# LauraFJulia/TFT_vs_Fund

Measured on NVIDIA B200. Metric: 3-view linear TFT pose solves/sec (LinearTFTPoseEstimation + ReprError, n=20), higher is better.
Workload: dtype f64

## Files before the change

### tft_vs_fund_b200/csrc/tvf_math.cuh

```cuda
#pragma once
#include <math.h>

#if defined(__CUDACC__)
#define TVF_HD __host__ __device__ __forceinline__
#else
#define TVF_HD inline
#endif

namespace tvf {

#ifndef TVF_FAST_RSQRT
#define TVF_FAST_RSQRT 1
#endif
#ifndef TVF_DLT_PREDICT
#define TVF_DLT_PREDICT 1
#endif

TVF_HD double rsqrt_(double x) {
#if defined(__CUDA_ARCH__)
#if TVF_FAST_RSQRT
    double y;
    asm("rsqrt.approx.ftz.f64 %0, %1;" : "=d"(y) : "d"(x));
    const double h = 0.5 * x;
    double e = fma(-h * y, y, 0.5);
// ... 183 lines not shown
    const double tiny = 1e-300 + 1e-18 * rmax;
    double d[3];
#pragma unroll
    for (int k = 0; k < 3; ++k) {
        const double p = (fabs(rr[k][k]) < tiny) ? copysign(tiny, rr[k][k]) : rr[k][k];
        d[k] = rcp_(p);
    }
    double x2 = d[2];
    double x1 = -(rr[1][2] * x2) * d[1];
    double x0 = -(rr[0][1] * x1 + rr[0][2] * x2) * d[0];
    double inv = rsqrt_(x0 * x0 + x1 * x1 + x2 * x2);
    x0 *= inv; x1 *= inv; x2 *= inv;
    double dprev = 0.0;
    bool ok = false;
    for (int it = 0; it < NULL3_MAX_IT; ++it) {
        const double y0 = x0 * d[0];
        const double y1 = (x1 - rr[0][1] * y0) * d[1];
        const double y2 = (x2 - rr[0][2] * y0 - rr[1][2] * y1) * d[2];
        double z2 = y2 * d[2];
        double z1 = (y1 - rr[1][2] * z2) * d[1];
        double z0 = (y0 - rr[0][1] * z1 - rr[0][2] * z2) * d[0];
        inv = rsqrt_(z0 * z0 + z1 * z1 + z2 * z2);
        z0 *= inv; z1 *= inv; z2 *= inv;
        const double e0 = z0 - x0, e1 = z1 - x1, e2 = z2 - x2;
        const double d2 = e0 * e0 + e1 * e1 + e2 * e2;
        x0 = z0; x1 = z1; x2 = z2;
        if (!(d2 > 1e-26) || !(d2 * d2 > 1e-28 * dprev)) { ok = (d2 == d2); break; }
        dprev = d2;
    }
    v[0] = x0; v[1] = x1; v[2] = x2;
    return ok;
}

TVF_HD void null3(const double* M, double* v) {
#if TVF_NULL3_QR
    if (null3_qr(M, false, v)) return;
#endif
    double A[9], V[9], s[3];
#pragma unroll
    for (int i = 0; i < 9; ++i) A[i] = M[i];
    jacobi_svd3(A, V, s);
    v[0] = V[6]; v[1] = V[7]; v[2] = V[8];
}
TVF_HD void null3_t(const double* M, double* v) {
#if TVF_NULL3_QR
    if (null3_qr(M, true, v)) return;
#endif
    double A[9], V[9], s[3];
#pragma unroll
    for (int c = 0; c < 3; ++c)
#pragma unroll
        for (int r = 0; r < 3; ++r) A[r + 3 * c] = M[c + 3 * r];
    jacobi_svd3(A, V, s);
    v[0] = V[6]; v[1] = V[7]; v[2] = V[8];
}

TVF_HD void svd3_full(const double* M, double* U, double* s, double* V) {
    double A[9];
#pragma unroll
    for (int i = 0; i < 9; ++i) A[i] = M[i];
    jacobi_svd3(A, V, s);
    const double i0 = rcp_(s[0]), i1 = rcp_(s[1]);
#pragma unroll
    for (int i = 0; i < 3; ++i) { U[i] = A[i] * i0; U[3 + i] = A[3 + i] * i1; }
    cross3(U, U + 3, U + 6);
}

TVF_HD void epipole_from_nulls(const double* v0, const double* v1, const double* v2, double* e) {
    double M[9];
#pragma unroll
    for (int c = 0; c < 3; ++c) { M[0 + 3 * c] = v0[c]; M[1 + 3 * c] = v1[c]; M[2 + 3 * c] = v2[c]; }
    null3(M, e);
}

TVF_HD void tft_epipoles(const double* T, double* e21, double* e31) {
    double v[9];
    null3(T, v); null3(T + 9, v + 3); null3(T + 18, v + 6);
    epipole_from_nulls(v, v + 3, v + 6, e31);
    null3_t(T, v); null3_t(T + 9, v + 3); null3_t(T + 18, v + 6);
    epipole_from_nulls(v, v + 3, v + 6, e21);
}

TVF_HD void onb3(const double* e, double* u1, double* u2) {
    const double sg = copysign(1.0, e[2]);
    const double a = -rcp_(sg + e[2]);
    const double b = e[0] * e[1] * a;
    u1[0] = 1.0 + sg * e[0] * e[0] * a; u1[1] = sg * b; u1[2] = -sg * e[0];
    u2[0] = b; u2[1] = sg + e[1] * e[1] * a; u2[2] = -e[1];
}

TVF_HD void transform_tft(const double* T, const double* M1, const double* M2, const double* M3,
                          int inverse, double* Tn) {
    double A1[9], A2[9], A3[9];
    if (inverse) {
#pragma unroll
        for (int i = 0; i < 9; ++i) A1[i] = M1[i];
        inv3(M2, A2); inv3(M3, A3);
    } else {
        inv3(M1, A1);
#pragma unroll
        for (int i = 0; i < 9; ++i) { A2[i] = M2[i]; A3[i] = M3[i]; }
    }
    double nrm = 0.0;
#pragma unroll
    for (int i = 0; i < 3; ++i) {
        double S[9], L[9];
#pragma unroll
        for (int e = 0; e < 9; ++e)
            S[e] = A1[0 + 3 * i] * T[e] + A1[1 + 3 * i] * T[9 + e] + A1[2 + 3 * i] * T[18 + e];
        mat3_mul(A2, S, L);
        mat3_mul_nt(L, A3, Tn + 9 * i);
#pragma unroll
        for (int e = 0; e < 9; ++e) nrm += Tn[9 * i + e] * Tn[9 * i + e];
    }
    const double inv = 1.0 / sqrt(nrm);
#pragma unroll
    for (int e = 0; e < 27; ++e) Tn[e] *= inv;
}

TVF_HD double det4_rows(const double* a, const double* b, const double* c, const double* d) {
    const double s0 = a[0] * b[1] - a[1] * b[0], s1 = a[0] * b[2] - a[2] * b[0];
    const double s2 = a[0] * b[3] - a[3] * b[0], s3 = a[1] * b[2] - a[2] * b[1];
    const double s4 = a[1] * b[3] - a[3] * b[1], s5 = a[2] * b[3] - a[3] * b[2];
    const double c5 = c[2] * d[3] - c[3] * d[2], c4 = c[1] * d[3] - c[3] * d[1];
    const double c3 = c[1] * d[2] - c[2] * d[1], c2 = c[0] * d[3] - c[3] * d[0];
    const double c1 = c[0] * d[2] - c[2] * d[0], c0 = c[0] * d[1] - c[1] * d[0];
    return s0 * c5 - s1 * c4 + s2 * c3 + s3 * c2 - s4 * c1 + s5 * c0;
}

TVF_HD void tft_from_p(const double* P1, const double* P2, const double* P3, double* T) {
    double r1[3][4], r2[3][4], r3[3][4];
#pragma unroll
    for (int r = 0; r < 3; ++r)
#pragma unroll
        for (int c = 0; c < 4; ++c) { r1[r][c] = P1[r + 3 * c]; r2[r][c] = P2[r + 3 * c]; r3[r][c] = P3[r + 3 * c]; }
    double nrm = 0.0;
#pragma unroll
    for (int i = 0; i < 3; ++i) {
        const int ra = (i == 0) ? 1 : 0, rb = (i == 2) ? 1 : 2;
        const double sg = (i == 1) ? -1.0 : 1.0;
#pragma unroll
        for (int j = 0; j < 3; ++j)
#pragma unroll
            for (int k = 0; k < 3; ++k) {
                const double d = sg * det4_rows(r1[ra], r1[rb], r2[j], r3[k]);
                T[j + 3 * k + 9 * i] = d; nrm += d * d;
            }
    }
    const double inv = 1.0 / sqrt(nrm);
#pragma unroll
    for (int e = 0; e < 27; ++e) T[e] *= inv;
}

template <int M>
TVF_HD void dlt_null(double (&a)[M][4], double* x, int* iters = nullptr) {
    double r[4][4];
#pragma unroll
    for (int k = 0; k < 4; ++k) {
        if (M == 4 && k == 3) {
            r[3][3] = -a[3][3];
            break;
        }
        double sig = 0.0;
#pragma unroll
        for (int i = k; i < M; ++i) sig += a[i][k] * a[i][k];
        const double nrm = sqrt_(sig);
        const double x1 = a[k][k];
        const double alpha = -copysign(nrm, x1);
        const double den = sig - alpha * x1;
        const double f = (den > 0.0) ? rcp_(den) : 0.0;
        const double vk = x1 - alpha;
#pragma unroll
        for (int c = k + 1; c < 4; ++c) {
            double sdot = vk * a[k][c];
#pragma unroll
            for (int i = k + 1; i < M; ++i) sdot += a[i][k] * a[i][c];
            sdot *= f;
            a[k][c] -= sdot * vk;
#pragma unroll
            for (int i = k + 1; i < M; ++i) a[i][c] -= sdot * a[i][k];
        }
        r[k][k] = alpha;
#pragma unroll
        for (int c = k + 1; c < 4; ++c) r[k][c] = a[k][c];
    }
    const double rmax = fmax(fmax(fabs(r[0][0]), fabs(r[1][1])), fmax(fabs(r[2][2]), fabs(r[3][3])));
    const double tiny = 1e-300 + 1e-18 * rmax;
    double d[4];
#pragma unroll
    for (int k = 0; k < 4; ++k) {
        const double p = (fabs(r[k][k]) < tiny) ? copysign(tiny, r[k][k]) : r[k][k];
        d[k] = rcp_(p);
    }
    double x0, x1, x2, x3;
    x3 = d[3];
    x2 = -(r[2][3] * x3) * d[2];
    x1 = -(r[1][2] * x2 + r[1][3] * x3) * d[1];
    x0 = -(r[0][1] * x1 + r[0][2] * x2 + r[0][3] * x3) * d[0];
    double inv = rsqrt_(x0 * x0 + x1 * x1 + x2 * x2 + x3 * x3);
    x0 *= inv; x1 *= inv; x2 *= inv; x3 *= inv;
    int it = 0;
#if TVF_DLT_PREDICT
    double dprev = 0.0;
#endif
    for (; it < 40; ++it) {
        const double y0 = x0 * d[0];
        const double y1 = (x1 - r[0][1] * y0) * d[1];
        const double y2 = (x2 - r[0][2] * y0 - r[1][2] * y1) * d[2];
        const double y3 = (x3 - r[0][3] * y0 - r[1][3] * y1 - r[2][3] * y2) * d[3];
        double z3 = y3 * d[3];
        double z2 = (y2 - r[2][3] * z3) * d[2];
        double z1 = (y1 - r[1][2] * z2 - r[1][3] * z3) * d[1];
        double z0 = (y0 - r[0][1] * z1 - r[0][2] * z2 - r[0][3] * z3) * d[0];
        inv = rsqrt_(z0 * z0 + z1 * z1 + z2 * z2 + z3 * z3);
        z0 *= inv; z1 *= inv; z2 *= inv; z3 *= inv;
#if TVF_DLT_PREDICT
        const double e0 = z0 - x0, e1 = z1 - x1, e2 = z2 - x2, e3 = z3 - x3;
        const double d2 = e0 * e0 + e1 * e1 + e2 * e2 + e3 * e3;
        x0 = z0; x1 = z1; x2 = z2; x3 = z3;
        if (!(d2 > 1e-26) || !(d2 * d2 > 1e-28 * dprev)) { ++it; break; }
        dprev = d2;
#else
        const double diff = fmax(fmax(fabs(z0 - x0), fabs(z1 - x1)), fmax(fabs(z2 - x2), fabs(z3 - x3)));
        x0 = z0; x1 = z1; x2 = z2; x3 = z3;
        if (!(diff > 1e-13)) { ++it; break; }
#endif
    }
    x[0] = x0; x[1] = x1; x[2] = x2; x[3] = x3;
    if (iters) *iters = it;
}

TVF_HD bool dlt4_depth_signs(const double (&a)[4][4], const double* r3, double tz, int* s_x, int* s_z) {
    double g[4][4];
#pragma unroll
    for (int i = 0; i < 4; ++i)
#pragma unroll
        for (int j = 0; j <= i; ++j) g[i][j] = a[0][i] * a[0][j] + a[1][i] * a[1][j] + a[2][i] * a[2][j] + a[3][i] * a[3][j];
    const double gmax = fmax(fmax(g[0][0], g[1][1]), fmax(g[2][2], g[3][3]));
    const double pmin = 1.0e-3 * gmax;
    if (!(g[0][0] >= pmin)) return false;
    const double i0 = rsqrt_(g[0][0]);
    const double l10 = g[1][0] * i0, l20 = g[2][0] * i0, l30 = g[3][0] * i0;
    const double p1 = g[1][1] - l10 * l10;
    if (!(p1 >= pmin)) return false;
    const double i1 = rsqrt_(p1);
    const double l21 = (g[2][1] - l20 * l10) * i1, l31 = (g[3][1] - l30 * l10) * i1;
    const double p2 = g[2][2] - l20 * l20 - l21 * l21;
    if (!(p2 >= pmin)) return false;
    const double i2 = rsqrt_(p2);
    const double l32 = (g[3][2] - l30 * l20 - l31 * l21) * i2;
    double p3 = g[3][3] - l30 * l30 - l31 * l31 - l32 * l32;
    p3 = (p3 >= 1.0e-14 * gmax) ? p3 : 1.0e-14 * gmax;
    const double i3 = rsqrt_(p3);
    double x3 = i3;
    double x2 = -(l32 * x3) * i2;
    double x1 = -(l21 * x2 + l31 * x3) * i1;
    double x0 = -(l10 * x1 + l20 * x2 + l30 * x3) * i0;
    double inv = rsqrt_(x0 * x0 + x1 * x1 + x2 * x2 + x3 * x3);
    x0 *= inv; x1 *= inv; x2 *= inv; x3 *= inv;
    double d2 = 1.0;
#pragma unroll
    for (int it = 0; it < 2; ++it) {
        const double y0 = x0 * i0;
        const double y1 = (x1 - l10 * y0) * i1;
        const double y2 = (x2 - l20 * y0 - l21 * y1) * i2;
        const double y3 = (x3 - l30 * y0 - l31 * y1 - l32 * y2) * i3;
        double z3 = y3 * i3;
        double z2 = (y2 - l32 * z3) * i2;
        double z1 = (y1 - l21 * z2 - l31 * z3) * i1;
        double z0 = (y0 - l10 * z1 - l20 * z2 - l30 * z3) * i0;
        inv = rsqrt_(z0 * z0 + z1 * z1 + z2 * z2 + z3 * z3);
        z0 *= inv; z1 *= inv; z2 *= inv; z3 *= inv;
        const double e0 = z0 - x0, e1 = z1 - x1, e2 = z2 - x2, e3 = z3 - x3;
        d2 = e0 * e0 + e1 * e1 + e2 * e2 + e3 * e3;
        x0 = z0; x1 = z1; x2 = z2; x3 = z3;
        if (d2 <= 1.0e-10) break;
    }
    if (!(d2 <= 1.0e-10)) return false;
    const double q1 = x2 * x3;
    const double zc = r3[0] * x0 + r3[1] * x1 + r3[2] * x2 + tz * x3;
    const double q2 = zc * x3;
    if (!(fabs(q1) >= 1.0e-3) || !(fabs(q2) >= 1.0e-3)) return false;
    *s_x = (q1 > 0.0) ? 1 : -1;
    *s_z = (q2 > 0.0) ? 1 : -1;
    return true;
}

template <bool AFF = false>
TVF_HD void dlt_row_minors(const double* ra, const double* rb, double* m7) {
    m7[0] = ra[0] * rb[1] - ra[1] * rb[0]; m7[1] = ra[0] * rb[2] - ra[2] * rb[0];
    m7[3] = ra[1] * rb[2] - ra[2] * rb[1];
    if (AFF) {
        m7[2] = 0.0; m7[4] = 0.0; m7[5] = 0.0;
        m7[6] = (ra[0] * ra[0] + ra[1] * ra[1] + ra[2] * ra[2]) + (rb[0] * rb[0] + rb[1] * rb[1] + rb[2] * rb[2]);
    } else {
        m7[2] = ra[0] * rb[3] - ra[3] * rb[0]; m7[4] = ra[1] * rb[3] - ra[3] * rb[1]; m7[5] = ra[2] * rb[3] - ra[3] * rb[2];
        m7[6] = (ra[0] * ra[0] + ra[1] * ra[1] + ra[2] * ra[2] + ra[3] * ra[3]) + (rb[0] * rb[0] + rb[1] * rb[1] + rb[2] * rb[2] + rb[3] * rb[3]);
    }
}
template <bool AFF = false>
TVF_HD bool dlt4_depth_signs_ray(const double* m7, const double* rc, const double* rd, const double* r3, double tz,
                                 int* s_x, int* s_z) {
    const double M01 = m7[0], M02 = m7[1], M03 = m7[2], M12 = m7[3], M13 = m7[4], M23 = m7[5];
    const double X0 = AFF ? rc[3] * M12 : rc[1] * M23 - rc[2] * M13 + rc[3] * M12;
    const double X1 = AFF ? -(rc[3] * M02) : -(rc[0] * M23 - rc[2] * M03 + rc[3] * M02);
    const double X2 = AFF ? rc[3] * M01 : rc[0] * M13 - rc[1] * M03 + rc[3] * M01;
    const double X3 = -(rc[0] * M12 - rc[1] * M02 + rc[2] * M01);
    const double xx = X0 * X0 + X1 * X1 + X2 * X2 + X3 * X3;
    const double b2 = m7[6] + (rc[0] * rc[0] + rc[1] * rc[1] + rc[2] * rc[2] + rc[3] * rc[3]);
    const double rho = rd[0] * X0 + rd[1] * X1 + rd[2] * X2 + rd[3] * X3;
    const double rb2 = fabs(rho) * b2;
    if (!(rb2 < 0.4 * xx)) return false;
    if (!(xx >= 1.0e-12 * (b2 * b2 * b2))) return false;
    const double q1 = X2 * X3;
    const double zc = r3[0] * X0 + r3[1] * X1 + r3[2] * X2 + tz * X3;
    const double q2 = zc * X3;
    const double floor_ = 1.0e-6 * xx;
    if (!(fabs(q1) >= 1.0605 * rb2 + floor_)) return false;
    if (!(fabs(q2) >= 1.616 * rb2 + floor_)) return false;
    *s_x = (q1 > 0.0) ? 1 : -1;
    *s_z = (q2 > 0.0) ? 1 : -1;
    return true;
}

TVF_HD void dlt_rows(const double* P, double x, double y, double* row_a, double* row_b) {
#pragma unroll
    for (int c = 0; c < 4; ++c) {
        row_a[c] = y * P[2 + 3 * c] - P[1 + 3 * c];
        row_b[c] = P[0 + 3 * c] - x * P[2 + 3 * c];
    }
}

TVF_HD void cam_apply(const double* P, const double* X, double* out) {
#pragma unroll
    for (int r = 0; r < 3; ++r)
        out[r] = P[r] * X[0] + P[r + 3] * X[1] + P[r + 6] * X[2] + P[r + 9] * X[3];
}

TVF_HD void decompose_essential(const double* E, double* R, double* Rp, double* t) {
    double U[9], s[3], V[9];
    svd3_full(E, U, s, V);
    double UW[9], UWt[9];
#pragma unroll
    for (int i = 0; i < 3; ++i) {
        UW[i] = U[3 + i]; UW[3 + i] = -U[i]; UW[6 + i] = U[6 + i];
        UWt[i] = -U[3 + i]; UWt[3 + i] = U[i]; UWt[6 + i] = U[6 + i];
    }
    mat3_mul_nt(UW, V, R);
    mat3_mul_nt(UWt, V, Rp);
    const double sr = sign_(det3(R)), sp = sign_(det3(Rp));
#pragma unroll
    for (int i = 0; i < 9; ++i) { R[i] *= sr; Rp[i] *= sp; }
    t[0] = U[6]; t[1] = U[7]; t[2] = U[8];
}

TVF_HD double matlab_abs_acos(double x) {
    if (x > 1.0) return log(x + sqrt(x * x - 1.0));
    if (x < -1.0) {
        const double a = log(-x + sqrt(x * x - 1.0));
        return sqrt(3.14159265358979323846 * 3.14159265358979323846 + a * a);
    }
    return acos(x);
}

TVF_HD void ang_error(const double* Rt_true, const double* Rt_est, double* rot_err, double* t_err) {
    double tr = 0.0;
#pragma unroll
    for (int i = 0; i < 9; ++i) tr += Rt_true[i] * Rt_est[i];
    const double k = 180.0 / 3.14159265358979323846;
    *rot_err = fabs(k * matlab_abs_acos((tr - 1.0) / 2.0));
    const double* a = Rt_est + 9; const double* b = Rt_true + 9;
    const double na = sqrt(a[0] * a[0] + a[1] * a[1] + a[2] * a[2]);
    const double nb = sqrt(b[0] * b[0] + b[1] * b[1] + b[2] * b[2]);
    const double d = (a[0] / na) * (b[0] / nb) + (a[1] / na) * (b[1] / nb) + (a[2] / na) * (b[2] / nb);
    *t_err = fabs(k * matlab_abs_acos(d));
}

}
```

### tft_vs_fund_b200/csrc/tvf_pose.cuh

```cuda
#pragma once
#include "tvf_math.cuh"

#ifndef TVF_CHEIR_UNROLL
#define TVF_CHEIR_UNROLL 1
#endif
#ifndef TVF_VOTE_FAST_SIGNS
#define TVF_VOTE_FAST_SIGNS 1
#endif
#ifndef TVF_VOTE_GRAM_SIGNS
#define TVF_VOTE_GRAM_SIGNS 0
#endif
#ifndef TVF_VOTE_RAY_SIGNS
#define TVF_VOTE_RAY_SIGNS 1
#endif
#ifndef TVF_CHEIR_NOINLINE
#define TVF_CHEIR_NOINLINE 0
#endif

namespace tvf {

constexpr int CAND_PAIR = 42;
constexpr int CAND_SIZE = 2 * CAND_PAIR;
constexpr int OFF_R = 0, OFF_RP = 9, OFF_T = 18, OFF_KR = 21, OFF_KRP = 30, OFF_KT = 39;

constexpr int ST_EIG_NOCONV = 1;
constexpr int ST_EPIPOLE_ZERO = 2;
constexpr int ST_NO_POSE_2 = 4;
constexpr int ST_NO_POSE_3 = 8;
constexpr int ST_NONFINITE = 16;

TVF_HD void fill_pair_(const double* E, const double* K, double* c) {
    decompose_essential(E, c + OFF_R, c + OFF_RP, c + OFF_T);
    mat3_mul(K, c + OFF_R, c + OFF_KR);
    mat3_mul(K, c + OFF_RP, c + OFF_KRP);
    mat3_vec(K, c + OFF_T, c + OFF_KT);
}

TVF_HD int candidates_from_tft(const double* T, const double* CalM, double* cand) {
    double K1[9], K2[9], K3[9];
#pragma unroll
    for (int c = 0; c < 3; ++c)
#pragma unroll
        for (int r = 0; r < 3; ++r) {
            K1[r + 3 * c] = CalM[r + 9 * c]; K2[r + 3 * c] = CalM[3 + r + 9 * c]; K3[r + 3 * c] = CalM[6 + r + 9 * c];
        }
    double Tc[27];
    transform_tft(T, K1, K2, K3, 1, Tc);
    double e21[3], e31[3];
    tft_epipoles(Tc, e21, e31);
    int st = 0;
    const double s31 = sign_(e31[2]), s21 = sign_(e21[2]);
    if (s31 == 0.0 || s21 == 0.0) st |= ST_EPIPOLE_ZERO;
#pragma unroll
    for (int i = 0; i < 3; ++i) { e31[i] *= s31; e21[i] *= s21; }
    double E21[9], E31[9];
#pragma unroll
    for (int i = 0; i < 3; ++i) {
        double a[3], b[3];
        mat3_vec(Tc + 9 * i, e31, a);
        cross3(e21, a, E21 + 3 * i);
        mat3_tvec(Tc + 9 * i, e21, b);
        cross3(e31, b, E31 + 3 * i);
        E31[3 * i] = -E31[3 * i]; E31[3 * i + 1] = -E31[3 * i + 1]; E31[3 * i + 2] = -E31[3 * i + 2];
    }
    fill_pair_(E21, K2, cand);
    fill_pair_(E31, K3, cand + CAND_PAIR);
    return st;
}

TVF_HD int candidates_from_f(const double* F21, const double* F31, const double* CalM, double* cand) {
    double K1[9], K2[9], K3[9];
#pragma unroll
    for (int c = 0; c < 3; ++c)
#pragma unroll
        for (int r = 0; r < 3; ++r) {
            K1[r + 3 * c] = CalM[r + 9 * c]; K2[r + 3 * c] = CalM[3 + r + 9 * c]; K3[r + 3 * c] = CalM[6 + r + 9 * c];
        }
    double tmp[9], E[9];
    mat3_mul_tn(K2, F21, tmp); mat3_mul(tmp, K1, E);
    fill_pair_(E, K2, cand);
    mat3_mul_tn(K3, F31, tmp); mat3_mul(tmp, K1, E);
    fill_pair_(E, K3, cand + CAND_PAIR);
    return 0;
}

TVF_HD void load_K1_as_P1(const double* CalM, double* P1) {
#pragma unroll
    for (int c = 0; c < 3; ++c)
#pragma unroll
        for (int r = 0; r < 3; ++r) P1[r + 3 * c] = CalM[r + 9 * c];
    P1[9] = 0.0; P1[10] = 0.0; P1[11] = 0.0;
}

TVF_HD void candidate_camera(const double* c, int k, double* P, double* r3, double* tz) {
    const double* KR = (k < 2) ? c + OFF_KR : c + OFF_KRP;
    const double* R = (k < 2) ? c + OFF_R : c + OFF_RP;
    const double sg = (k == 0 || k == 3) ? 1.0 : -1.0;
#pragma unroll
    for (int i = 0; i < 9; ++i) P[i] = KR[i];
    P[9] = sg * c[OFF_KT]; P[10] = sg * c[OFF_KT + 1]; P[11] = sg * c[OFF_KT + 2];
    r3[0] = R[2]; r3[1] = R[5]; r3[2] = R[8];
    *tz = sg * c[OFF_T + 2];
}

TVF_HD void triangulate2(const double* Pa, const double* Pb, double xa, double ya, double xb, double yb, double* X) {
    double a[4][4];
    dlt_rows(Pa, xa, ya, a[0], a[1]);
    dlt_rows(Pb, xb, yb, a[2], a[3]);
    dlt_null<4>(a, X);
}

TVF_HD void triangulate3(const double* Pa, const double* Pb, const double* Pc, const double* p6, double* X) {
    double a[6][4];
    dlt_rows(Pa, p6[0], p6[1], a[0], a[1]);
    dlt_rows(Pb, p6[2], p6[3], a[2], a[3]);
    dlt_rows(Pc, p6[4], p6[5], a[4], a[5]);
    dlt_null<6>(a, X);
}

#if defined(__CUDACC__) && TVF_CHEIR_NOINLINE
#define TVF_COLD_DEV __host__ __device__ __noinline__ static
#else
#define TVF_COLD_DEV TVF_HD
#endif
TVF_COLD_DEV void cheirality_accurate(const double* ra, const double* rb, const double* rc, const double* rd, const double* r3,
                                      double tz, int q, int* v, int* nanmask, double* dst) {
    double a[4][4];
#pragma unroll
    for (int e = 0; e < 4; ++e) { a[0][e] = ra[e]; a[1][e] = rb[e]; a[2][e] = rc[e]; a[3][e] = rd[e]; }
#if TVF_VOTE_FAST_SIGNS && TVF_VOTE_GRAM_SIGNS
    if (dst == nullptr) {
        int sx, sz;
        if (dlt4_depth_signs(a, r3, tz, &sx, &sz)) { v[q] += sx + sz; return; }
    }
#endif
    double X[4];
    dlt_null<4>(a, X);
    const double iw = (X[3] != 0.0) ? rcp_(X[3]) : 1.0 / X[3];
    const double X0 = X[0] * iw, X1 = X[1] * iw, X2 = X[2] * iw, X3 = X[3] * iw;
    const double z2 = r3[0] * X0 + r3[1] * X1 + r3[2] * X2 + tz * X3;
    if (X2 != X2 || z2 != z2) {
        *nanmask |= (1 << q);
    } else {
        v[q] += (int)sign_(X2) + (int)sign_(z2);
    }
    if (dst != nullptr) { dst[0] = X[0]; dst[1] = X[1]; dst[2] = X[2]; dst[3] = X[3]; }
}

template <bool AFF = false>
TVF_HD void cheirality_point(const double* ra, const double* rb, const double* m7, const double* c, double x2, double y2,
                             int* v, int* nanmask, double* Xa, double* Xb) {
    constexpr int kUnroll = TVF_CHEIR_UNROLL;
#pragma unroll(kUnroll)
    for (int q = 0; q < 2; ++q) {
        double P[12], r3[3], tz;
        candidate_camera(c, q == 0 ? 0 : 3, P, r3, &tz);
        double rc[4], rd[4];
        dlt_rows(P, x2, y2, rc, rd);
        double* dst = (q == 0) ? Xa : Xb;
#if TVF_VOTE_FAST_SIGNS && TVF_VOTE_RAY_SIGNS
        if (dst == nullptr) {
            int sx, sz;
            if (m7 != nullptr && dlt4_depth_signs_ray<AFF>(m7, rc, rd, r3, tz, &sx, &sz)) { v[q] += sx + sz; continue; }
        }
#endif
        cheirality_accurate(ra, rb, rc, rd, r3, tz, q, v, nanmask, dst);
    }
}

TVF_HD void expand_votes(const int* v2, int nan2, int* vote4, int* nan4) {
    vote4[0] = v2[0]; vote4[1] = -v2[0]; vote4[2] = -v2[1]; vote4[3] = v2[1];
    *nan4 = ((nan2 & 1) ? 3 : 0) | ((nan2 & 2) ? 12 : 0);
}

TVF_HD int select_candidate(const int* vote, int nanmask) {
    int best = 0, sel = -1;
#pragma unroll
    for (int k = 0; k < 4; ++k) {
        if (!((nanmask >> k) & 1) && vote[k] >= best) { sel = k; best = vote[k]; }
    }
    return sel;
}

TVF_HD void selected_pose(const double* c, int k, double* Rt, double* P) {
    const double* R = (k < 2) ? c + OFF_R : c + OFF_RP;
    const double* KR = (k < 2) ? c + OFF_KR : c + OFF_KRP;
    const double sg = (k == 0 || k == 3) ? 1.0 : -1.0;
#pragma unroll
    for (int i = 0; i < 9; ++i) { Rt[i] = R[i]; P[i] = KR[i]; }
#pragma unroll
    for (int i = 0; i < 3; ++i) { Rt[9 + i] = sg * c[OFF_T + i]; P[9 + i] = sg * c[OFF_KT + i]; }
}

TVF_HD void scale_point(const double* P1, const double* P2, const double* KR3, const double* u3,
                        const double* p6, double* num, double* den) {
    double X[4];
    triangulate2(P1, P2, p6[0], p6[1], p6[2], p6[3], X);
    const double iw = 1.0 / X[3];
    const double Xc[3] = {X[0] * iw, X[1] * iw, X[2] * iw};
    double X3[3];
    mat3_vec(KR3, Xc, X3);
    const double p3[3] = {p6[4], p6[5], 1.0};
    double c1[3], c2[3];
    cross3(p3, X3, c1);
    cross3(p3, u3, c2);
    *num = c1[0] * c2[0] + c1[1] * c2[1] + c1[2] * c2[2];
    *den = c2[0] * c2[0] + c2[1] * c2[1] + c2[2] * c2[2];
}

TVF_HD double final_point(const double* P1, const double* P2, const double* P3, const double* p6, double* Xout) {
    double X[4];
    triangulate3(P1, P2, P3, p6, X);
    const double iw = 1.0 / X[3];
    const double Xe[4] = {X[0] * iw, X[1] * iw, X[2] * iw, 1.0};
    Xout[0] = Xe[0]; Xout[1] = Xe[1]; Xout[2] = Xe[2];
    double sq = 0.0;
    const double* Ps[3] = {P1, P2, P3};
#pragma unroll
    for (int v = 0; v < 3; ++v) {
        double x[3];
        cam_apply(Ps[v], Xe, x);
        const double iz = 1.0 / x[2];
        const double dx = x[0] * iz - p6[2 * v], dy = x[1] * iz - p6[2 * v + 1];
        sq += dx * dx + dy * dy;
    }
    return sq;
}

TVF_HD double final_point_kt(const double* P1, const double* P2, const double* P3, const double* t3s, const double* p6,
                             double* Xout) {
    double a[6][4];
    dlt_rows(P1, p6[0], p6[1], a[0], a[1]);
    dlt_rows(P2, p6[2], p6[3], a[2], a[3]);
#pragma unroll
    for (int c = 0; c < 3; ++c) {
        a[4][c] = p6[5] * P3[2 + 3 * c] - P3[1 + 3 * c];
        a[5][c] = P3[0 + 3 * c] - p6[4] * P3[2 + 3 * c];
    }
    a[4][3] = p6[5] * t3s[2] - t3s[1];
    a[5][3] = t3s[0] - p6[4] * t3s[2];
    double X[4];
    dlt_null<6>(a, X);
    const double iw = 1.0 / X[3];
    const double Xe[4] = {X[0] * iw, X[1] * iw, X[2] * iw, 1.0};
    Xout[0] = Xe[0]; Xout[1] = Xe[1]; Xout[2] = Xe[2];
    double sq = 0.0;
#pragma unroll
    for (int v = 0; v < 3; ++v) {
        double x[3];
        if (v < 2) {
            cam_apply(v == 0 ? P1 : P2, Xe, x);
        } else {
#pragma unroll
            for (int r = 0; r < 3; ++r) x[r] = P3[r] * Xe[0] + P3[r + 3] * Xe[1] + P3[r + 6] * Xe[2] + t3s[r] * Xe[3];
        }
        const double iz = 1.0 / x[2];
        const double dx = x[0] * iz - p6[2 * v], dy = x[1] * iz - p6[2 * v + 1];
        sq += dx * dx + dy * dy;
    }
    return sq;
}

}
```

### tft_vs_fund_b200/csrc/tvf_pose_kernels.cu

```cuda
#include "tvf_kernels.h"
#include "tvf_pose.cuh"
#include "tvf_async.cuh"

namespace tvf {

constexpr int PT_THREADS = 256;

struct PointMap {
    int ppb;
    int tpp;
    int lp;
    int lpt;
    __device__ __forceinline__ PointMap(int n, int threads = PT_THREADS) {
        tpp = (n <= threads) ? n : threads;
        ppb = threads / tpp;
        lp = threadIdx.x / tpp;
        lpt = threadIdx.x - lp * tpp;
    }
};

#ifndef TVF_TAIL_SERIAL_SUM
#define TVF_TAIL_SERIAL_SUM 1
#endif

// ... 321 lines not shown

#ifndef TVF_TAIL_MINB
#define TVF_TAIL_MINB 2
#endif
#ifndef TVF_TAIL_REUSE_X
#define TVF_TAIL_REUSE_X 0
#endif
#ifndef TVF_TAIL_TMA
#define TVF_TAIL_TMA 1
#endif
__device__ __forceinline__ double camera_entry(const double* calm, const double* cand, int k2, int k3, int i) {
    if (i < 12) return (i < 9) ? calm[(i % 3) + 9 * (i / 3)] : 0.0;
    const int pair = (i >= 24) ? 1 : 0, e = i - 12 - 12 * pair, k = pair ? k3 : k2;
    const double* c = cand + pair * CAND_PAIR;
    if (e < 9) return c[((k < 2) ? OFF_KR : OFF_KRP) + e];
    return ((k == 0 || k == 3) ? 1.0 : -1.0) * c[OFF_KT + e - 9];
}
__device__ __forceinline__ double pose_entry(const double* c, int k, int i) {
    if (i < 9) return c[((k < 2) ? OFF_R : OFF_RP) + i];
    return ((k == 0 || k == 3) ? 1.0 : -1.0) * c[OFF_T + i - 9];
}
__device__ __forceinline__ void seg_reduce2_split(double* ra, double* rb, const PointMap& m) {
    if (m.tpp > 32) { seg_reduce2(ra, rb, m); return; }
    __syncthreads();
    if (m.lp < m.ppb && m.lpt < 2) {
        double* r = (m.lpt ? rb : ra) + (threadIdx.x - m.lpt);
        double acc = r[0];
        for (int i = 1; i < m.tpp; ++i) acc += r[i];
        r[0] = acc;
    }
    __syncthreads();
}
__device__ __forceinline__ void seg_reduce1(double* ra, const PointMap& m) {
    if (m.tpp > 32) { seg_reduce(ra, m); return; }
    __syncthreads();
    if (m.lp < m.ppb && m.lpt == 0) {
        double* r = ra + threadIdx.x;
        double acc = r[0];
        for (int i = 1; i < m.tpp; ++i) acc += r[i];
        r[0] = acc;
    }
}

#ifndef TVF_TAIL_CTA
#define TVF_TAIL_CTA 128
#endif
#ifndef TVF_TAIL_MINB_SMALL
#define TVF_TAIL_MINB_SMALL ((TVF_TAIL_MINB * PT_THREADS) / TVF_TAIL_CTA)
#endif
template <int THREADS>
__global__ void __launch_bounds__(THREADS, THREADS == PT_THREADS ? TVF_TAIL_MINB : TVF_TAIL_MINB_SMALL)
pose_tail_fused_kernel(PoseTailArgs a) {
    constexpr int MAX_PPB = THREADS / TAIL_FUSED_MIN_N;
    constexpr int PT_THREADS = THREADS;
    __shared__ int sv[MAX_PPB * 4];
    __shared__ int snan[MAX_PPB];
    __shared__ double sP[MAX_PPB * 36];
    __shared__ double red0[THREADS], red1[THREADS], red2[THREADS];
    const PointMap m(a.n, THREADS);
    const int own = threadIdx.x - m.lpt;
    const double qnan = __longlong_as_double(0x7ff8000000000000LL);
#if TVF_TAIL_TMA
    extern __shared__ __align__(16) unsigned char tail_dsm[];
    __shared__ unsigned long long tbar[2];
    const unsigned pts_bytes = (unsigned)m.ppb * (unsigned)a.n * 48u, cand_bytes = (unsigned)m.ppb * (unsigned)(CAND_SIZE * 8);
    const unsigned stage_bytes = pts_bytes + cand_bytes;
    const long long bstep = (long long)gridDim.x * m.ppb;
    auto issue = [&](long long b0n, int stage) {
        const long long left = a.B - b0n;
        const unsigned np = (unsigned)(left < m.ppb ? left : m.ppb);
        unsigned char* dst = tail_dsm + (size_t)stage * stage_bytes;
        mbar_expect_tx(&tbar[stage], np * (unsigned)a.n * 48u + np * (unsigned)(CAND_SIZE * 8));
        bulk_g2s(dst, a.corresp + b0n * a.n * 6, np * (unsigned)a.n * 48u, &tbar[stage]);
        bulk_g2s(dst + pts_bytes, a.cand + b0n * CAND_SIZE, np * (unsigned)(CAND_SIZE * 8), &tbar[stage]);
    };
    if (threadIdx.x == 0) {
        mbar_init(&tbar[0], 1); mbar_init(&tbar[1], 1);
        asm volatile("fence.mbarrier_init.release.cluster;" ::: "memory");
    }
#endif
    for (int e = threadIdx.x; e < m.ppb * 4; e += PT_THREADS) sv[e] = 0;
    for (int e = threadIdx.x; e < m.ppb; e += PT_THREADS) snan[e] = 0;
    __syncthreads();
#if TVF_TAIL_TMA
    if (threadIdx.x == 0 && (long long)blockIdx.x * m.ppb < a.B) issue((long long)blockIdx.x * m.ppb, 0);
    int iter = 0;
#endif
    for (long long b0 = (long long)blockIdx.x * m.ppb; b0 < a.B; b0 += (long long)gridDim.x * m.ppb) {
        const long long b = b0 + m.lp;
        const bool live = (m.lp < m.ppb && b < a.B);
#if TVF_TAIL_TMA
        if (threadIdx.x == 0 && b0 + bstep < a.B) issue(b0 + bstep, (iter + 1) & 1);
        const unsigned char* stg = tail_dsm + (size_t)(iter & 1) * stage_bytes;
        mbar_wait(&tbar[iter & 1], (unsigned)(iter >> 1) & 1u);
        ++iter;
        const double* cand = reinterpret_cast<const double*>(stg + pts_bytes) + (live ? m.lp : 0) * CAND_SIZE;
#else
        const double* cand = a.cand + (live ? b : 0) * CAND_SIZE;
#endif
        double* Ps = sP + (live ? m.lp : 0) * 36;
        double p6[6] = {0, 0, 0, 0, 0, 0};
#if TVF_TAIL_REUSE_X
        double Xa[4] = {0, 0, 0, 1}, Xb[4] = {0, 0, 0, 1};
#endif
        if (live) {
            double P1[12];
            load_K1_as_P1(calm_of(a, b), P1);
#if TVF_TAIL_TMA
            const double2* q = reinterpret_cast<const double2*>(stg) + (m.lp * a.n + m.lpt) * 3;
            const double2 q1 = q[0], q2 = q[1], q3 = q[2];
#else
            const double2* q = reinterpret_cast<const double2*>(a.corresp + (b * a.n + m.lpt) * 6);
            const double2 q1 = __ldg(q), q2 = __ldg(q + 1), q3 = __ldg(q + 2);
#endif
            p6[0] = q1.x; p6[1] = q1.y; p6[2] = q2.x; p6[3] = q2.y; p6[4] = q3.x; p6[5] = q3.y;
            double ra[4], rb[4], m7[7];
            dlt_rows(P1, p6[0], p6[1], ra, rb);
            dlt_row_minors<TVF_RAY_AFF>(ra, rb, m7);
            int v2[2] = {0, 0}, v3[2] = {0, 0}, n2 = 0, n3 = 0;
#if TVF_TAIL_REUSE_X
            cheirality_point<TVF_RAY_AFF>(ra, rb, m7, cand, p6[2], p6[3], v2, &n2, Xa, Xb);
#else
            cheirality_point<TVF_RAY_AFF>(ra, rb, m7, cand, p6[2], p6[3], v2, &n2, nullptr, nullptr);
#endif
            cheirality_point<TVF_RAY_AFF>(ra, rb, m7, cand + CAND_PAIR, p6[4], p6[5], v3, &n3, nullptr, nullptr);
            int* dst = sv + m.lp * 4;
            if (v2[0]) atomicAdd(dst + 0, v2[0]);
            if (v2[1]) atomicAdd(dst + 1, v2[1]);
            if (v3[0]) atomicAdd(dst + 2, v3[0]);
            if (v3[1]) atomicAdd(dst + 3, v3[1]);
            if (n2 | n3) atomicOr(snan + m.lp, n2 | (n3 << 2));
        }
        __syncthreads();
        int k2 = 15, k3 = 15;
        if (live) {
            int vote[8], nan2, nan3;
            expand_votes(sv + m.lp * 4, snan[m.lp] & 3, vote, &nan2);
            expand_votes(sv + m.lp * 4 + 2, (snan[m.lp] >> 2) & 3, vote + 4, &nan3);
            const int s2 = select_candidate(vote, nan2), s3 = select_candidate(vote + 4, nan3);
            k2 = (s2 < 0) ? 15 : s2; k3 = (s3 < 0) ? 15 : s3;
            if (m.lpt == 0 && a.votes != nullptr) {
                int* gv = a.votes + b * 10;
#pragma unroll
                for (int k = 0; k < 8; ++k) gv[k] = vote[k];
                gv[8] = nan2; gv[9] = nan3;
            }
            const double* calm = calm_of(a, b);
            for (int i = m.lpt; i < 36; i += m.tpp) Ps[i] = camera_entry(calm, cand, s2 < 0 ? 0 : s2, s3 < 0 ? 0 : s3, i);
        }
        __syncthreads();
        for (int e = threadIdx.x; e < m.ppb * 4; e += PT_THREADS) sv[e] = 0;
        for (int e = threadIdx.x; e < m.ppb; e += PT_THREADS) snan[e] = 0;
        double num = 0.0, den = 0.0;
        if (live) {
#if TVF_TAIL_REUSE_X
            const bool useA = (k2 == 0 || k2 == 1 || k2 == 15);
            const double w = ((k2 == 1 || k2 == 2) ? -1.0 : 1.0) * (useA ? Xa[3] : Xb[3]);
            const double iw = 1.0 / w;
            const double Xc[3] = {(useA ? Xa[0] : Xb[0]) * iw, (useA ? Xa[1] : Xb[1]) * iw, (useA ? Xa[2] : Xb[2]) * iw};
            double X3[3], c1[3], c2[3];
            mat3_vec(Ps + 24, Xc, X3);
            const double p3[3] = {p6[4], p6[5], 1.0};
            cross3(p3, X3, c1);
            cross3(p3, Ps + 33, c2);
            num = c1[0] * c2[0] + c1[1] * c2[1] + c1[2] * c2[2];
            den = c2[0] * c2[0] + c2[1] * c2[1] + c2[2] * c2[2];
#else
            scale_point(Ps, Ps + 12, Ps + 24, Ps + 33, p6, &num, &den);
#endif
        }
        red0[threadIdx.x] = num; red1[threadIdx.x] = den;
        seg_reduce2_split(red0, red1, m);
        const bool ok = (k2 != 15) && (k3 != 15);
        double sq = 0.0;
        if (live) {
            const double snum = red0[own], sden = red1[own];
            const double lam = -snum / sden;
            bool fin = true;
            const int kk2 = (k2 == 15) ? 0 : k2, kk3 = (k3 == 15) ? 0 : k3;
            for (int i = m.lpt; i < 12; i += m.tpp) {
                const double r2 = pose_entry(cand, kk2, i);
                double r3 = pose_entry(cand + CAND_PAIR, kk3, i);
                if (i >= 9) r3 *= lam;
                fin = fin && isfinite(r2) && isfinite(r3);
                if (a.Rt2 != nullptr) a.Rt2[b * 12 + i] = ok ? r2 : qnan;
                if (a.Rt3 != nullptr) a.Rt3[b * 12 + i] = ok ? r3 : qnan;
            }
            int st = fin ? 0 : ST_NONFINITE;
            if (m.lpt == 0) {
                if (a.scale != nullptr) { a.scale[2 * b] = snum; a.scale[2 * b + 1] = sden; }
                if (k2 == 15) st |= ST_NO_POSE_2;
                if (k3 == 15) st |= ST_NO_POSE_3;
            }
            if (a.status != nullptr && st != 0) atomicOr(a.status + b, st);
            const double t3s[3] = {Ps[33] * lam, Ps[34] * lam, Ps[35] * lam};
            double X[3];
            sq = final_point_kt(Ps, Ps + 12, Ps + 24, t3s, p6, X);
            if (a.reconst != nullptr) {
                double* dst = a.reconst + (b * a.n + m.lpt) * 3;
                dst[0] = ok ? X[0] : qnan; dst[1] = ok ? X[1] : qnan; dst[2] = ok ? X[2] : qnan;
            }
        }
        red2[threadIdx.x] = sq;
        seg_reduce1(red2, m);
        if (live && m.lpt == 0) {
            const double err = sqrt(red2[threadIdx.x] / (3.0 * (double)a.n));
            if (a.repr_err != nullptr) a.repr_err[b] = ok ? err : qnan;
            if (a.status != nullptr && !isfinite(err)) atomicOr(a.status + b, ST_NONFINITE);
        }
    }
}

__global__ void __launch_bounds__(128)
tft_from_pose_kernel(const double* __restrict__ calm, int calm_batched, const double* __restrict__ Rt2,
                     const double* __restrict__ Rt3, long long B, double* __restrict__ T) {
    const long long b = (long long)blockIdx.x * blockDim.x + threadIdx.x;
    if (b >= B) return;
    const double* cm = calm + (calm_batched ? b * 27 : 0);
    double K[3][9];
#pragma unroll
    for (int v = 0; v < 3; ++v)
#pragma unroll
        for (int c = 0; c < 3; ++c)
#pragma unroll
            for (int r = 0; r < 3; ++r) K[v][r + 3 * c] = __ldg(cm + 3 * v + r + 9 * c);
    double P1[12], P2[12], P3[12], R[12];
#pragma unroll
    for (int i = 0; i < 9; ++i) P1[i] = K[0][i];
    P1[9] = 0.0; P1[10] = 0.0; P1[11] = 0.0;
#pragma unroll
    for (int i = 0; i < 12; ++i) R[i] = Rt2[b * 12 + i];
    mat3_mul(K[1], R, P2); mat3_vec(K[1], R + 9, P2 + 9);
#pragma unroll
    for (int i = 0; i < 12; ++i) R[i] = Rt3[b * 12 + i];
    mat3_mul(K[2], R, P3); mat3_vec(K[2], R + 9, P3 + 9);
    double t[27];
    tft_from_p(P1, P2, P3, t);
#pragma unroll
    for (int i = 0; i < 27; ++i) T[b * 27 + i] = t[i];
}

__global__ void normalize2d_kernel(const double* __restrict__ pts, int n, long long B, double* __restrict__ out,
                                   double* __restrict__ Nmat) {
    const int lane = threadIdx.x & 31;
    const long long b = ((long long)blockIdx.x * blockDim.x + threadIdx.x) >> 5;
    if (b >= B) return;
    const double* p = pts + b * 2 * n;
    double sx = 0.0, sy = 0.0;
    for (int i = lane; i < n; i += 32) { sx += p[2 * i]; sy += p[2 * i + 1]; }
#pragma unroll
    for (int o = 16; o > 0; o >>= 1) { sx += __shfl_xor_sync(0xffffffffu, sx, o); sy += __shfl_xor_sync(0xffffffffu, sy, o); }
    const double cx = sx / n, cy = sy / n;
    double d = 0.0;
    for (int i = lane; i < n; i += 32) { const double dx = p[2 * i] - cx, dy = p[2 * i + 1] - cy; d += sqrt(dx * dx + dy * dy); }
#pragma unroll
    for (int o = 16; o > 0; o >>= 1) d += __shfl_xor_sync(0xffffffffu, d, o);
    const double s = 1.4142135623730951 / (d / n);
    const double tx = -s * cx, ty = -s * cy;
    if (out != nullptr)
        for (int i = lane; i < n; i += 32) { out[b * 2 * n + 2 * i] = s * p[2 * i] + tx; out[b * 2 * n + 2 * i + 1] = s * p[2 * i + 1] + ty; }
    if (Nmat != nullptr && lane == 0) {
        double* N = Nmat + b * 9;
        N[0] = s; N[1] = 0; N[2] = 0; N[3] = 0; N[4] = s; N[5] = 0; N[6] = tx; N[7] = ty; N[8] = 1.0;
    }
}

__global__ void transform_tft_kernel(const double* __restrict__ T, const double* __restrict__ M1,
                                     const double* __restrict__ M2, const double* __restrict__ M3, int mats_batched,
                                     int inverse, long long B, double* __restrict__ Tout) {
    const long long b = (long long)blockIdx.x * blockDim.x + threadIdx.x;
    if (b >= B) return;
    const long long mo = mats_batched ? b * 9 : 0;
    double t[27], m1[9], m2[9], m3[9], o[27];
#pragma unroll
    for (int i = 0; i < 27; ++i) t[i] = T[b * 27 + i];
#pragma unroll
    for (int i = 0; i < 9; ++i) { m1[i] = M1[mo + i]; m2[i] = M2[mo + i]; m3[i] = M3[mo + i]; }
    transform_tft(t, m1, m2, m3, inverse, o);
#pragma unroll
    for (int i = 0; i < 27; ++i) Tout[b * 27 + i] = o[i];
}

__global__ void tft_from_p_kernel(const double* __restrict__ P1, const double* __restrict__ P2,
                                  const double* __restrict__ P3, long long B, double* __restrict__ T) {
    const long long b = (long long)blockIdx.x * blockDim.x + threadIdx.x;
    if (b >= B) return;
    double a[12], c[12], d[12], t[27];
#pragma unroll
    for (int i = 0; i < 12; ++i) { a[i] = P1[b * 12 + i]; c[i] = P2[b * 12 + i]; d[i] = P3[b * 12 + i]; }
    tft_from_p(a, c, d, t);
#pragma unroll
    for (int i = 0; i < 27; ++i) T[b * 27 + i] = t[i];
}

__device__ __forceinline__ void load_xy(const double* pts, int M, int rows, int n, long long b, int pt, int v,
                                        double* x, double* y) {
    const double* p = pts + ((b * n + pt) * M + v) * rows;
    double px = p[0], py = p[1];
    if (rows == 3) { const double w = p[2]; px /= w; py /= w; }
    *x = px; *y = py;
}

template <int M>
__device__ __forceinline__ void triangulate_m(const double* P, const double* pts, int rows, int n, long long b, int pt,
                                              double* X) {
    double a[2 * M][4];
#pragma unroll
    for (int v = 0; v < M; ++v) {
        double x, y;
        load_xy(pts, M, rows, n, b, pt, v, &x, &y);
        dlt_rows(P + 12 * v, x, y, a[2 * v], a[2 * v + 1]);
    }
    dlt_null<2 * M>(a, X);
}

__global__ void triangulate_kernel(const double* __restrict__ P, int M, int cams_batched, const double* __restrict__ pts,
                                   int rows, int n, long long B, double* __restrict__ X) {
    const long long e = (long long)blockIdx.x * blockDim.x + threadIdx.x;
    if (e >= B * n) return;
    const long long b = e / n;
    const int pt = (int)(e - b * n);
    const double* Pb = P + (cams_batched ? b * 12 * M : 0);
    double x[4];
    if (M == 2) triangulate_m<2>(Pb, pts, rows, n, b, pt, x);
    else triangulate_m<3>(Pb, pts, rows, n, b, pt, x);
#pragma unroll
    for (int i = 0; i < 4; ++i) X[e * 4 + i] = x[i];
}

__global__ void __launch_bounds__(PT_THREADS)
repr_error_kernel(const double* __restrict__ P, int M, int cams_batched, const double* __restrict__ corresp, int rows,
                  int n, long long B, const double* __restrict__ pts3d, int pts_rows, double* __restrict__ err) {
    __shared__ double rsq[PT_THREADS];
    const PointMap m(n);
    for (long long b0 = (long long)blockIdx.x * m.ppb; b0 < B; b0 += (long long)gridDim.x * m.ppb) {
        const long long b = b0 + m.lp;
        const bool live = (m.lp < m.ppb && b < B);
        double sq = 0.0;
        if (live) {
            const double* Pb = P + (cams_batched ? b * 12 * M : 0);
            for (int pt = m.lpt; pt < n; pt += m.tpp) {
                double X[4];
                if (pts3d == nullptr) {
                    if (M == 2) triangulate_m<2>(Pb, corresp, rows, n, b, pt, X);
                    else triangulate_m<3>(Pb, corresp, rows, n, b, pt, X);
                } else {
                    const double* q = pts3d + (b * n + pt) * pts_rows;
                    X[0] = q[0]; X[1] = q[1]; X[2] = q[2]; X[3] = (pts_rows == 4) ? q[3] : 1.0;
                }
                for (int v = 0; v < M; ++v) {
// ... 223 lines not shown
```

Measured before the change: 109.7 million.

## Reuse two-view QR factor for three-view triangulation via rank-2 update

The two-view DLT triangulation now keeps its R factor and null vector. The final three-view triangulation reuses them: it folds the two third-camera rows into the existing R with a Householder update and warm-starts inverse iteration from the two-view solution, instead of factoring a fresh 6x4 system. The first camera's known zero translation entry (P1 = [K|0]) is also skipped in the first Householder step. This trades some register pressure from carrying the factor struct, plus a small change in the numerical path, for fewer FLOPs and fewer inverse-iteration steps per point. When TVF_TAIL_REUSE_X is on, the extra two-view triangulation is recomputed just to build the factor, which could cancel the savings.

```diff
diff --git a/tft_vs_fund_b200/csrc/tvf_math.cuh b/tft_vs_fund_b200/csrc/tvf_math.cuh
--- a/tft_vs_fund_b200/csrc/tvf_math.cuh
+++ b/tft_vs_fund_b200/csrc/tvf_math.cuh
@@ -359,9 +359,19 @@
     for (int e = 0; e < 27; ++e) T[e] *= inv;
 }
 
-template <int M>
-TVF_HD void dlt_null(double (&a)[M][4], double* x, int* iters = nullptr) {
-    double r[4][4];
+
+TVF_HD void dlt_pivots(const double (&r)[4][4], double (&d)[4]) {
+    const double rmax = fmax(fmax(fabs(r[0][0]), fabs(r[1][1])), fmax(fabs(r[2][2]), fabs(r[3][3])));
+    const double tiny = 1e-300 + 1e-18 * rmax;
+#pragma unroll
+    for (int k = 0; k < 4; ++k) {
+        const double p = (fabs(r[k][k]) < tiny) ? copysign(tiny, r[k][k]) : r[k][k];
+        d[k] = rcp_(p);
+    }
+}
+
+template <int M, bool AFF = false>
+TVF_HD void dlt_qr(double (&a)[M][4], double (&r)[4][4], double (&d)[4]) {
 #pragma unroll
     for (int k = 0; k < 4; ++k) {
         if (M == 4 && k == 3) {
@@ -379,33 +389,58 @@
         const double vk = x1 - alpha;
 #pragma unroll
         for (int c = k + 1; c < 4; ++c) {
-            double sdot = vk * a[k][c];
-#pragma unroll
-            for (int i = k + 1; i < M; ++i) sdot += a[i][k] * a[i][c];
+            const bool z = AFF && k == 0 && c == 3;
+            double sdot = z ? 0.0 : vk * a[k][c];
+#pragma unroll
+            for (int i = k + 1; i < M; ++i)
+                if (!(z && i == 1)) sdot += a[i][k] * a[i][c];
             sdot *= f;
-            a[k][c] -= sdot * vk;
-#pragma unroll
-            for (int i = k + 1; i < M; ++i) a[i][c] -= sdot * a[i][k];
+            a[k][c] = z ? -(sdot * vk) : a[k][c] - sdot * vk;
+#pragma unroll
+            for (int i = k + 1; i < M; ++i) a[i][c] = (z && i == 1) ? -(sdot * a[i][k]) : a[i][c] - sdot * a[i][k];
         }
         r[k][k] = alpha;
 #pragma unroll
         for (int c = k + 1; c < 4; ++c) r[k][c] = a[k][c];
     }
-    const double rmax = fmax(fmax(fabs(r[0][0]), fabs(r[1][1])), fmax(fabs(r[2][2]), fabs(r[3][3])));
-    const double tiny = 1e-300 + 1e-18 * rmax;
-    double d[4];
+    dlt_pivots(r, d);
+}
+
+TVF_HD void dlt_qr_add2(double (&r)[4][4], double (&b)[2][4], double (&d)[4]) {
 #pragma unroll
     for (int k = 0; k < 4; ++k) {
-        const double p = (fabs(r[k][k]) < tiny) ? copysign(tiny, r[k][k]) : r[k][k];
-        d[k] = rcp_(p);
-    }
+        const double sig = r[k][k] * r[k][k] + b[0][k] * b[0][k] + b[1][k] * b[1][k];
+        const double nrm = sqrt_(sig);
+        const double x1 = r[k][k];
+        const double alpha = -copysign(nrm, x1);
+        const double den = sig - alpha * x1;
+        const double f = (den > 0.0) ? rcp_(den) : 0.0;
+        const double vk = x1 - alpha;
+#pragma unroll
+        for (int c = k + 1; c < 4; ++c) {
+            double sdot = vk * r[k][c] + b[0][k] * b[0][c] + b[1][k] * b[1][c];
+            sdot *= f;
+            r[k][c] -= sdot * vk;
+            b[0][c] -= sdot * b[0][k];
+            b[1][c] -= sdot * b[1][k];
+        }
+        r[k][k] = alpha;
+    }
+    dlt_pivots(r, d);
+}
+
+TVF_HD void dlt_start_e4(const double (&r)[4][4], const double (&d)[4], double* x) {
     double x0, x1, x2, x3;
     x3 = d[3];
     x2 = -(r[2][3] * x3) * d[2];
     x1 = -(r[1][2] * x2 + r[1][3] * x3) * d[1];
     x0 = -(r[0][1] * x1 + r[0][2] * x2 + r[0][3] * x3) * d[0];
-    double inv = rsqrt_(x0 * x0 + x1 * x1 + x2 * x2 + x3 * x3);
-    x0 *= inv; x1 *= inv; x2 *= inv; x3 *= inv;
+    const double inv = rsqrt_(x0 * x0 + x1 * x1 + x2 * x2 + x3 * x3);
+    x[0] = x0 * inv; x[1] = x1 * inv; x[2] = x2 * inv; x[3] = x3 * inv;
+}
+
+TVF_HD int dlt_inverse_iteration(const double (&r)[4][4], const double (&d)[4], double* x) {
+    double x0 = x[0], x1 = x[1], x2 = x[2], x3 = x[3], inv;
     int it = 0;
 #if TVF_DLT_PREDICT
     double dprev = 0.0;
@@ -434,6 +469,15 @@
 #endif
     }
     x[0] = x0; x[1] = x1; x[2] = x2; x[3] = x3;
+    return it;
+}
+
+template <int M>
+TVF_HD void dlt_null(double (&a)[M][4], double* x, int* iters = nullptr) {
+    double r[4][4], d[4];
+    dlt_qr<M>(a, r, d);
+    dlt_start_e4(r, d, x);
+    const int it = dlt_inverse_iteration(r, d, x);
     if (iters) *iters = it;
 }
 
diff --git a/tft_vs_fund_b200/csrc/tvf_pose.cuh b/tft_vs_fund_b200/csrc/tvf_pose.cuh
--- a/tft_vs_fund_b200/csrc/tvf_pose.cuh
+++ b/tft_vs_fund_b200/csrc/tvf_pose.cuh
@@ -103,11 +103,18 @@
     *tz = sg * c[OFF_T + 2];
 }
 
-TVF_HD void triangulate2(const double* Pa, const double* Pb, double xa, double ya, double xb, double yb, double* X) {
-    double a[4][4];
-    dlt_rows(Pa, xa, ya, a[0], a[1]);
-    dlt_rows(Pb, xb, yb, a[2], a[3]);
-    dlt_null<4>(a, X);
+struct DltFactor2 {
+    double r[4][4];
+    double x[4];
+};
+
+TVF_HD void triangulate2_k1(const double* P1, const double* P2, const double* p6, DltFactor2& f) {
+    double a[4][4], d[4];
+    dlt_rows(P1, p6[0], p6[1], a[0], a[1]);
+    dlt_rows(P2, p6[2], p6[3], a[2], a[3]);
+    dlt_qr<4, true>(a, f.r, d);
+    dlt_start_e4(f.r, d, f.x);
+    dlt_inverse_iteration(f.r, d, f.x);
 }
 
 TVF_HD void triangulate3(const double* Pa, const double* Pb, const double* Pc, const double* p6, double* X) {
@@ -193,9 +200,11 @@
 }
 
 TVF_HD void scale_point(const double* P1, const double* P2, const double* KR3, const double* u3,
-                        const double* p6, double* num, double* den) {
-    double X[4];
-    triangulate2(P1, P2, p6[0], p6[1], p6[2], p6[3], X);
+                        const double* p6, double* num, double* den, DltFactor2* keep = nullptr) {
+    DltFactor2 f;
+    triangulate2_k1(P1, P2, p6, f);
+    const double* X = f.x;
+    if (keep != nullptr) *keep = f;
     const double iw = 1.0 / X[3];
     const double Xc[3] = {X[0] * iw, X[1] * iw, X[2] * iw};
     double X3[3];
@@ -228,19 +237,19 @@
 }
 
 TVF_HD double final_point_kt(const double* P1, const double* P2, const double* P3, const double* t3s, const double* p6,
-                             double* Xout) {
-    double a[6][4];
-    dlt_rows(P1, p6[0], p6[1], a[0], a[1]);
-    dlt_rows(P2, p6[2], p6[3], a[2], a[3]);
+                             DltFactor2& f, double* Xout) {
+    double b[2][4], d[4];
 #pragma unroll
     for (int c = 0; c < 3; ++c) {
-        a[4][c] = p6[5] * P3[2 + 3 * c] - P3[1 + 3 * c];
-        a[5][c] = P3[0 + 3 * c] - p6[4] * P3[2 + 3 * c];
-    }
-    a[4][3] = p6[5] * t3s[2] - t3s[1];
-    a[5][3] = t3s[0] - p6[4] * t3s[2];
-    double X[4];
-    dlt_null<6>(a, X);
+        b[0][c] = p6[5] * P3[2 + 3 * c] - P3[1 + 3 * c];
+        b[1][c] = P3[0 + 3 * c] - p6[4] * P3[2 + 3 * c];
+    }
+    b[0][3] = p6[5] * t3s[2] - t3s[1];
+    b[1][3] = t3s[0] - p6[4] * t3s[2];
+    dlt_qr_add2(f.r, b, d);
+    double X[4] = {f.x[0], f.x[1], f.x[2], f.x[3]};
+    if (!(X[0] * X[0] + X[1] * X[1] + X[2] * X[2] + X[3] * X[3] > 0.5)) dlt_start_e4(f.r, d, X);
+    dlt_inverse_iteration(f.r, d, X);
     const double iw = 1.0 / X[3];
     const double Xe[4] = {X[0] * iw, X[1] * iw, X[2] * iw, 1.0};
     Xout[0] = Xe[0]; Xout[1] = Xe[1]; Xout[2] = Xe[2];
diff --git a/tft_vs_fund_b200/csrc/tvf_pose_kernels.cu b/tft_vs_fund_b200/csrc/tvf_pose_kernels.cu
--- a/tft_vs_fund_b200/csrc/tvf_pose_kernels.cu
+++ b/tft_vs_fund_b200/csrc/tvf_pose_kernels.cu
@@ -497,6 +497,7 @@
         for (int e = threadIdx.x; e < m.ppb * 4; e += PT_THREADS) sv[e] = 0;
         for (int e = threadIdx.x; e < m.ppb; e += PT_THREADS) snan[e] = 0;
         double num = 0.0, den = 0.0;
+        DltFactor2 fac;
         if (live) {
 #if TVF_TAIL_REUSE_X
             const bool useA = (k2 == 0 || k2 == 1 || k2 == 15);
@@ -510,8 +511,9 @@
             cross3(p3, Ps + 33, c2);
             num = c1[0] * c2[0] + c1[1] * c2[1] + c1[2] * c2[2];
             den = c2[0] * c2[0] + c2[1] * c2[1] + c2[2] * c2[2];
+            triangulate2_k1(Ps, Ps + 12, p6, fac);
 #else
-            scale_point(Ps, Ps + 12, Ps + 24, Ps + 33, p6, &num, &den);
+            scale_point(Ps, Ps + 12, Ps + 24, Ps + 33, p6, &num, &den, &fac);
 #endif
         }
         red0[threadIdx.x] = num; red1[threadIdx.x] = den;
@@ -540,7 +542,7 @@
             if (a.status != nullptr && st != 0) atomicOr(a.status + b, st);
             const double t3s[3] = {Ps[33] * lam, Ps[34] * lam, Ps[35] * lam};
             double X[3];
-            sq = final_point_kt(Ps, Ps + 12, Ps + 24, t3s, p6, X);
+            sq = final_point_kt(Ps, Ps + 12, Ps + 24, t3s, p6, fac, X);
             if (a.reconst != nullptr) {
                 double* dst = a.reconst + (b * a.n + m.lpt) * 3;
                 dst[0] = ok ? X[0] : qnan; dst[1] = ok ? X[1] : qnan; dst[2] = ok ? X[2] : qnan;
```

After: 111.6 million (median of 6 runs). 1.02x the previous value.
